# stevengiacalone/triceratops

Hardware: AMD Instinct MI355X
Metric: light-curve-point x sample evals/sec (higher is better)
Workload: dtype f64

## Files before the change

### include/trx_debug.h

```cpp
#ifndef TRX_DEBUG_H
#define TRX_DEBUG_H

#include "trx.h"

#ifdef __cplusplus
extern "C" {
#endif

int trx_set_rows_per_wave(int rows);
int trx_set_cell_packing_below(int n_time);
int trx_debug_batch_plan(long rows, int rows_per_wave, int taper, long* positions, int* rows_min);

int trx_set_supersample_tiers(int on);
int trx_set_stencil(int on);
int trx_set_skip_excluded(int on);
int trx_set_debug_node_counts(int on);
int trx_set_kepler_stepping(int on);

int trx_set_bounded_evaluation(int mode);
int trx_set_debug_bounded_lnl(int on);
int trx_set_debug_poison(int on);
int trx_set_debug_bug(int on);
int trx_set_probe_rows(int rows);
int trx_set_star_chain(int on);
int trx_set_row_order(int on);
int trx_debug_row_order(long* n_rows, long* segment_capacity, int* counts, int* lists, double* row_blocks);
int trx_set_whole_trips(int on);
int trx_set_one_sweep(int mode);
int trx_debug_whole_trips(long* whole, long* walked, int reset);
int trx_debug_chain_counts(long* chains, long* calls_in_chains, long* posterior_calls_in_chains, int reset);

int trx_debug_select_from_halfchi2(const double* halfchi2, const double* lnprior, const double* cols,
                                   const double* cols_pad, long n, long N, long n_total, int ncol, int twin, int K,
                                   int moments, double lnsigma, double* out_record, double* out_post_x,
                                   double* out_table, void* stream);

int trx_debug_capture_buffers(long* live, long* idle);

#ifdef __cplusplus
}
#endif
#endif
```

### triceratops_amd/_lib.py

```python
import ctypes
import os
import threading

import numpy as np
import torch

_HERE = os.path.dirname(os.path.abspath(__file__))
LIB_PATH = os.environ.get("TRX_LIB") or os.path.join(_HERE, "libtrx.so")
TESTING_LIB_PATH = os.environ.get("TRX_TESTING_LIB") or os.path.join(_HERE, "libtrx_testing.so")

MODEL_TP, MODEL_EB, MODEL_EB_TWIN, MODEL_RAW = 0, 1, 2, 3
FLAG_COMPANION_IS_HOST, FLAG_SCALAR_K, FLAG_FP32_MODEL, FLAG_EVALUATE_EXCLUDED = 1, 2, 4, 8
FLAG_ALL_SUBEXPOSURES, FLAG_NO_STENCIL, FLAG_COUNT_EVALUATIONS, FLAG_FULL_EVALUATION = 16, 32, 64, 128
FLAG_WEIGHT_MOMENTS = 256
N_PARAM = {MODEL_TP: 10, MODEL_EB: 11, MODEL_EB_TWIN: 11, MODEL_RAW: 9}
ERR_NTOTAL = 4

ABI_SYMBOLS = (
    "trx_lnl_batch", "trx_lnl_batch_weighted", "trx_flux_grid", "trx_chi2_grid", "trx_chi2_grid_weighted",
    "trx_chi2_grid_offset", "trx_chi2_grid_baseline", "trx_workspace_bytes",
    "trx_log_mean_exp", "trx_lnz_scenario", "trx_lnz_from_halfchi2", "trx_lnz_moments_from_halfchi2",
    "trx_posterior_from_halfchi2", "trx_grid_quantiles",
    "trx_lnl_batch_host", "trx_flux_grid_host",
    "trx_log_mean_exp_host", "trx_skipped_rows", "trx_pruned_rows",
    "trx_draw_scenario", "trx_draw_args_size", "trx_scenario_evidence", "trx_scenario_enqueue", "trx_star_enqueue",
    "trx_scenario_args_size", "trx_release_scratch", "trx_version", "trx_last_error", "trx_device_count",
)
WARP_SYMBOLS = ("trxw_hist_from_halfchi2",)
NOISE_SYMBOLS = ("trxn_chi2_grid_ou",)
MIX_SYMBOLS = ("trxm_chi2_grid_ou_mix",)
SHIFT_SYMBOLS = ("trxt_softmin_rows",)
ROBUST_SYMBOLS = ("trxr_chi2_grid_robust",)
GLS_SYMBOLS = ("trxg_chi2_grid_ou_baseline",)
SS_SYMBOLS = ("trxs_chi2_grid_ss2",)
DEBUG_SYMBOLS = (
    "trx_set_rows_per_wave", "trx_set_cell_packing_below", "trx_debug_batch_plan", "trx_set_supersample_tiers",
    "trx_set_stencil", "trx_set_skip_excluded", "trx_set_debug_node_counts", "trx_set_kepler_stepping",
    "trx_set_bounded_evaluation", "trx_set_debug_bounded_lnl", "trx_set_debug_poison", "trx_set_debug_bug",
    "trx_set_probe_rows", "trx_set_star_chain", "trx_debug_capture_buffers", "trx_debug_chain_counts",
    "trx_set_row_order", "trx_debug_row_order", "trx_set_whole_trips", "trx_debug_whole_trips", "trx_set_one_sweep",
    "trx_debug_select_from_halfchi2",
)


class TrxError(RuntimeError):
    pass


EXTRA_FLAGS = 0
CELL_PACKING_BELOW = 320
STATS = {"rows": 0, "cells": 0, "launches": 0, "native_calls": 0}
_stats_lock = threading.Lock()


def count_launch(rows, n_time):
    with _stats_lock:
        STATS["rows"] += rows
        STATS["cells"] += rows * n_time
        STATS["launches"] += 1
TRACE = None
TRACE_SAMPLE_ROWS = 128


def reset_stats():
    for k in STATS:
        STATS[k] = 0


def set_precision(mode):
    global EXTRA_FLAGS
    if mode not in ("fp64", "fp32"):
        raise ValueError("precision must be 'fp64' or 'fp32'")
    EXTRA_FLAGS = (EXTRA_FLAGS & ~FLAG_FP32_MODEL) | (FLAG_FP32_MODEL if mode == "fp32" else 0)

# ... 87 lines not shown
                                        _vp]
    L.trxt_softmin_rows.restype = c_int
    L.trxt_softmin_rows.argtypes = [_vp, c_long, c_long, c_int, _vp, c_int, _vp, _vp]
    L.trxr_chi2_grid_robust.restype = c_int
    L.trxr_chi2_grid_robust.argtypes = [_vp, _vp, _vp, c_int, c_long, _vp, c_double, c_int, _vp, c_double, c_double, c_double,
                                        _vp]
    L.trxg_chi2_grid_ou_baseline.restype = c_int
    L.trxg_chi2_grid_ou_baseline.argtypes = [_vp, _vp, c_int, c_long, _vp, c_double, c_int, _vp, _vp, _vp, _vp, _vp, c_int,
                                             _vp, _vp, _vp]
    L.trxs_chi2_grid_ss2.restype = c_int
    L.trxs_chi2_grid_ss2.argtypes = [_vp, _vp, c_int, c_long, _vp, c_double, c_int, _vp, _vp, _vp, _vp, _vp]
    L.trx_grid_quantiles.restype = c_int
    L.trx_grid_quantiles.argtypes = [_vp, c_long, c_int, _vp, _vp, c_long, _vp, c_int, _vp, _vp]
    L.trx_lnl_batch_host.restype = c_int
    L.trx_lnl_batch_host.argtypes = [c_int, c_int, _vp, _vp, c_int, c_double, _vp, c_long,
                                     c_double, c_int, _vp]
    L.trx_flux_grid_host.restype = c_int
    L.trx_flux_grid_host.argtypes = [c_int, c_int, _vp, c_int, _vp, c_long, c_double, c_int, _vp, _vp]
    L.trx_log_mean_exp_host.restype = c_int
    L.trx_log_mean_exp_host.argtypes = [_vp, c_long, c_long, _vp]
    L.trx_skipped_rows.restype = c_int
    L.trx_skipped_rows.argtypes = [ctypes.POINTER(ctypes.c_ulonglong), c_int]
    L.trx_pruned_rows.restype = c_int
    L.trx_pruned_rows.argtypes = [ctypes.POINTER(ctypes.c_ulonglong), c_int]
    L.trx_version.restype = ctypes.c_char_p
    L.trx_last_error.restype = ctypes.c_char_p
    L.trx_device_count.restype = c_int
    L.trx_testing = bool(testing)
    if testing:
        for name in ("trx_set_rows_per_wave", "trx_set_kepler_stepping", "trx_set_skip_excluded",
                     "trx_set_bounded_evaluation", "trx_set_debug_bounded_lnl", "trx_set_debug_poison",
                     "trx_set_debug_bug", "trx_set_star_chain", "trx_set_probe_rows", "trx_set_stencil",
                     "trx_set_supersample_tiers", "trx_set_debug_node_counts", "trx_set_cell_packing_below",
                     "trx_set_row_order", "trx_set_whole_trips", "trx_set_one_sweep"):
            fn = getattr(L, name)
            fn.restype = c_int
            fn.argtypes = [c_int]
        L.trx_debug_capture_buffers.restype = c_int
        L.trx_debug_capture_buffers.argtypes = [ctypes.POINTER(c_long), ctypes.POINTER(c_long)]
        L.trx_debug_row_order.restype = c_int
        L.trx_debug_row_order.argtypes = [ctypes.POINTER(c_long), ctypes.POINTER(c_long), _vp, _vp, _vp]
        L.trx_debug_whole_trips.restype = c_int
        L.trx_debug_whole_trips.argtypes = [ctypes.POINTER(c_long), ctypes.POINTER(c_long), c_int]
        L.trx_debug_select_from_halfchi2.restype = c_int
        L.trx_debug_select_from_halfchi2.argtypes = [_vp, _vp, _vp, _vp, c_long, c_long, c_long, c_int, c_int, c_int, c_int,
                                                     c_double, _vp, _vp, _vp, _vp]
    return L


def check(rc):
    if rc:
        msg = lib().trx_last_error().decode()
        if rc == ERR_NTOTAL:
            raise ValueError(msg)
        raise TrxError("libtrx error %d: %s" % (rc, msg))


def version():
    return lib().trx_version().decode()


_gpu_seen = False


def require_gpu():
    global _gpu_seen
    if _gpu_seen:
        return
    if not torch.cuda.is_available() or lib().trx_device_count() < 1:
        raise TrxError("triceratops_amd needs an AMD GPU (gfx950); none is visible and there is no "
# ... 475 lines not shown
```

### triceratops_amd/csrc/trx_cells.hpp

```cpp
#pragma once
#include <hip/hip_runtime.h>
#include <math.h>

#include <cstddef>
#include <cstdint>

#include "../../include/trx.h"
#include "trx_device.hpp"
#include "trx_internal.hpp"

namespace {

using namespace trx;

constexpr int MODE_LNL = 0;
constexpr int MODE_GRID = 1;

struct RowsArgs {
    int model, flags;
    const double* time;
    const double* flux;
    int n_time;
    double sigma;
    const double* params;
// ... 14 lines not shown
    int tl_off;
    int wave_off, wave_doubles;
    int probe_rows;
    int wave_floor;
    int wave_floor3;
    double* rowc;
    int* scan_list;
    unsigned long long* scan_count;
    const long* n_dev;
    const int* src_idx;
    long src_stride;
    int twin_cols;
    int dense;
    int forced_B;
    int prune;
    int pstride;
    int pstride3;
    double prune_c0;
    const double* prune_lp;
    int part;
    int split;
    int* surv_list;
    unsigned long long* surv_count;
    int* probe_list;
    unsigned long long* probe_count;
    TierHead tiers;
    const double* tier_xw;
    double s2, rs2, dS, rS;
    const double* inv_var;
    double sec_limit;
    int accumulate;
    int whole_trips;
    int one_sweep;
    int* order;
};

#ifndef TRX_CHAIN_MAX_BRANCHES
#define TRX_CHAIN_MAX_BRANCHES 24
#endif
struct BranchArgs {
    int model, flags, twin_cols, need_sec;
    const double* flux;
    double sigma, s2, rs2, prune_c0;
    const double* params;
    double* out;
    const long* n_dev;
    const int* src_idx;
    const double* prune_lp;
    double* scratch;
    unsigned long long* scan_count;
};
constexpr int kChainMaxBranches = TRX_CHAIN_MAX_BRANCHES;
struct BranchTab {
    BranchArgs b[kChainMaxBranches];
};
static_assert(sizeof(RowsArgs) + sizeof(BranchTab) + 16 <= 4096, "kernel argument buffer");

__device__ __forceinline__ double uniform(double v)
{
    const unsigned long long b = __double_as_longlong(v);
    const unsigned lo = __builtin_amdgcn_readfirstlane((unsigned)b);
    const unsigned hi = __builtin_amdgcn_readfirstlane((unsigned)(b >> 32));
    return __longlong_as_double(((unsigned long long)hi << 32) | lo);
}

__device__ __forceinline__ long uniform_long(long v)
// ... 20 lines not shown
    return __builtin_amdgcn_mbcnt_hi((unsigned)(m >> 32), __builtin_amdgcn_mbcnt_lo((unsigned)m, 0u));
}

#ifdef TRX_PHASE_TIMERS
__device__ unsigned long long g_phase_cycles[8];
#define TRX_TICK(var) const unsigned long long var = __builtin_readcyclecounter()
#define TRX_TOCK(slot, from) tm[slot] += __builtin_readcyclecounter() - (from)
#else
#define TRX_TICK(var)
#define TRX_TOCK(slot, from)
#endif

#ifdef TRX_TAIL_TIMERS
constexpr int kTailWaves = 1 << 17;
__device__ unsigned long long g_tail[4] = {~0ull, 0ull, 0ull, 0ull};
__device__ unsigned long long g_tail_finish[kTailWaves];
#endif

constexpr int kStatShards = 256, kStatPad = 16;
__device__ unsigned long long g_row_stats[2][kStatShards][kStatPad];
__device__ __forceinline__ void add_row_stat(int which, unsigned count)
{
    if (count) atomicAdd(&g_row_stats[which][(blockIdx.x + 41u * blockIdx.y) & (kStatShards - 1)][0], (unsigned long long)count);
}

#ifdef TRX_TESTING
__device__ unsigned long long g_trip_stats[2][kStatShards][kStatPad];
__device__ __forceinline__ void add_trip_stat(int which, unsigned count)
{
    if (count) atomicAdd(&g_trip_stats[which][(blockIdx.x + 41u * blockIdx.y) & (kStatShards - 1)][0], (unsigned long long)count);
}
__device__ __forceinline__ bool whole_trips_on(const RowsArgs& a) { return a.whole_trips != 0; }
__device__ __forceinline__ bool one_sweep_on(const RowsArgs& a, bool lnl) { return a.one_sweep >= (lnl ? 1 : 2); }
#define TRX_TRIP_STAT(var) ++var
#else
__device__ __forceinline__ bool whole_trips_on(const RowsArgs&) { return true; }
__device__ __forceinline__ bool one_sweep_on(const RowsArgs&, bool lnl) { return lnl; }
#define TRX_TRIP_STAT(var)
#endif

__device__ __forceinline__ double k_rule(double k, bool scalar_rule)
{
    if (scalar_rule) { if (fabs(k - 1.0) < 1e-6) k *= 0.999; }
    else             { if ((k - 1.0) < 1e-6) k *= 0.999; }
    return k;
}

#ifndef TRX_BATCH_WAVES
#define TRX_BATCH_WAVES 4
#endif

constexpr int kBatchWaves = TRX_BATCH_WAVES;
__host__ __device__ constexpr int cells_waves(bool long_rows) { return long_rows ? 1 : kBatchWaves; }
#ifndef TRX_TIER_LDS
#define TRX_TIER_LDS(PRUNE, LONG) true
#endif
#ifndef TRX_ATAN_TAB
#define TRX_ATAN_TAB(PRUNE, LONG) (((PRUNE) && !(LONG)) ? 2 : 1)
#endif
#ifndef TRX_LONG_ROWS_IN_LDS
#define TRX_LONG_ROWS_IN_LDS 0
#endif
#ifndef TRX_CARRY_CELLS
#define TRX_CARRY_CELLS 1
#endif
#ifndef TRX_CELLS_WAVES_PER_EU
#define TRX_CELLS_WAVES_PER_EU 4
#endif
#ifndef TRX_LAZY_TIERS
#define TRX_LAZY_TIERS 1
// ... 494 lines not shown
            double m = secnan[lane] ? NAN : secmin[lane];
            m = (m + ysec) / (1.0 + ysec);
            const double secdepth = 1.0 - (m + fdil) / (1.0 + fdil);
            a.rowc[row * kRowDoubles + (kRowDoubles - 1)] =
                (WT ? !(secdepth >= a.sec_limit) : (secdepth < 1.5 * a.sigma)) ? 0.0 : 1.0;
            if (a.out_sec) a.out_sec[row] = secdepth;
        }
        __syncthreads();
    }
}

template <int E, bool WT = false>
__global__ __launch_bounds__(64) void sec_scan_kernel(RowsArgs a)
{
    sec_scan_body<E, WT>(a);
}

struct BranchMap {
    unsigned char id[TRX_CHAIN_MAX_BRANCHES];
};
__global__ __launch_bounds__(64) void sec_scan_kernel_star(RowsArgs common, BranchTab bt, BranchMap map)
{
    const RowsArgs a = star_args(common, bt, 0, (int)map.id[blockIdx.y]);
    if (!a.need_sec) return;
    sec_scan_body<8>(a);
}
static_assert(offsetof(RowC, excl) == (kRowDoubles - 1) * sizeof(double), "excl is the last field of RowC");

struct CellState {
    double sE[64], cE[64];
    double t[64];
    double facc[64];
    unsigned meta[64];
    unsigned short rel[64];
};
struct StencilState {
    double fc[64 + ((kStM + 7) & ~7)];
    double stw[(2 * kStM + 1 + 7) & ~7];
};
constexpr int kCentreNode = 1023;

__device__ __forceinline__ double fp32_model_slack(double lb, int n_probed, double rs2)
{
    return 1e-5 * sqrt(2.0 * (double)n_probed * rs2 * fmax(lb, 0.0));
}

template <int BITS>
__device__ __forceinline__ int lane_prefix(int cnt, int& total)
{
    int off = 0;
    total = 0;
#pragma unroll
    for (int b = 0; b < BITS; ++b) {
        const unsigned long long m = __ballot((cnt >> b) & 1);
        off += lanes_below(m) << b;
        total += __popcll(m) << b;
    }
    return off;
}

__device__ __forceinline__ long row_order_at(const int* __restrict__ order, long v, long n, int lane)
{
    const int cnt = order[lane * kOrderStride];
    int incl = cnt;
#pragma unroll
    for (int o = 1; o < 64; o <<= 1) {
        const int up = __shfl_up(incl, o, 64);
        if (lane >= o) incl += up;
    }
    const long first = (long)(incl - cnt);
    const unsigned long long below = __ballot(cnt >= 0 && first <= v);
    const int seg = __popcll(below) - 1;
// ... 400 lines not shown
                    const double dMc = reduce_2pi(phase);
                    const double slack = 1e-15 * fabs(phase);
                    const RowC& cw = rows[rr];
                    inw = in_window(cw.wlo - slack, cw.whi + slack, dMc) && !mask_bit(skipmask, rr);
                    if (MODE == MODE_GRID && (!inw || a.debug_nodes))
                        a.out[(size_t)base * n_time + cell] = a.debug_nodes ? 0.0 : hmout[rr];
                    if (LONG && MODE == MODE_LNL && !inw && phase_no == 0) {
                        const double d = fl[j] - 1.0;
                        lacc = fma(d * d, WT ? wl[j] : rs2, lacc);
                    }
                    if (PRUNE) {
                        if (!LONG && inw && phase_no == 0) {
                            const double d = fl[j] - 1.0;
                            __hip_atomic_fetch_add(&hrem[rr], (d * d) * rs2, __ATOMIC_RELAXED, __HIP_MEMORY_SCOPE_WORKGROUP);
                        }
                        if (nphase == 2) {
                            const bool probe = (j % pstride) == (pstride >> 1);
                            inw = inw && (probe == (phase_no == 0));
                        }
                    }
                }
                const unsigned long long mw = __ballot(inw);
                if (inw) winlist[nw + lanes_below(mw)] = (unsigned short)(cell - win0);
                nw += __popcll(mw);
            }
            wave_sync();
            TRX_TOCK(1, t_p1);
            constexpr bool kOneSweep = TRX_ONE_SWEEP && (LONG || TRX_ONE_SWEEP_BATCH) && !PRUNE;
            const bool one = kOneSweep && one_sweep_on(a, MODE == MODE_LNL);
            int nheavy = 0;
            for (int sweep = 0; sweep < (one ? 1 : 2); ++sweep) {
            const int count = sweep ? nheavy : nw;
            const bool halo = ST && sweep == 0 && st_radius > 0.0;
            int carry_j = 0;
            unsigned long long carry_ok = 0;
            int ncarry = 0;
            for (int w0 = 0, step = 64; w0 < count || (kCarry && ncarry > 0); w0 += step) {
                TRX_TICK(t_plan);
                TRX_CENSUS_ADD(sweep ? kCenChunk1 : kCenChunk0, 1);
                bool owned = true;
                const bool carried = kCarry && lane < ncarry;
                if (kCarry) step = 64 - ncarry;
                const int csrc = (lane + 64 - ncarry) & 63;
                const unsigned cmeta = carried ? cs.meta[csrc] : 0u;
                bool valid = carried ? (cmeta & 0x20000u) != 0 : (w0 + lane - ncarry) < count;
                int rel = (int)*(carried ? &cs.rel[csrc] : &winlist[valid ? (w0 + lane - ncarry) : (count - 1)]);
                bool last_chunk = false;
                if (ST && halo) {
                    last_chunk = w0 + 64 >= count;
                    step = last_chunk ? 64 : 64 - kStM;
                    owned = lane < step;
                    if (w0 > 0 && lane < kStM) ss.fc[lane] = ss.fc[kStM + (64 - 2 * kStM) + lane];
                    wave_sync();
                }
                const int cell = win0 + rel;
                int rr = 0, j = cell;
                if (!LONG) {
                    rr = (int)(((float)cell + 0.5f) * inv_nt);
                    rr = rr < nb ? rr : nb - 1;
                    j = cell - rr * n_time;
                }
                const double t = tl[j];
                double fobs = 0.0;
                if (LONG && MODE == MODE_LNL) fobs = fl[j];
                double wobs = rs2;
                if (LONG && WT) wobs = wl[j];
                CellPlan pl;
                if (carried) {
                    pl.n = (int)(cmeta >> 18); pl.tier = (int)((cmeta >> 8) & 0xffu) - 1;
                    pl.sE = cs.sE[csrc]; pl.cE = cs.cE[csrc];
                    pl.anchored = (cmeta & 0x10000u) != 0;
                } else if (valid) {
                    const RowC& c = (LONG && !TRX_LONG_ROWS_IN_LDS) ? cu : rows[rr];
#ifndef TRX_PLAN_FULL_SOLVE
                    if (LONG && sweep == 1) pl = plan_all_subexposures<PRUNE>(c, t, a.S);
                    else
#endif
                    pl = plan_cell<false, PRUNE, TRX_TIER_LDS(PRUNE, LONG), kLazyTiers>(c, t, a.exptime, a.S, a.tiers, a.use_tiers != 0,
                                                                                        (ST && sweep == 0) ? st_radius : 0.0, thead);
                    if (STEP && !pl.anchored && pl.n > 0) {
                        kepler_full(c.nmot * (t - c.t0) + c.Mtr, c.e, pl.sE, pl.cE);
                        pl.anchored = true;
                    }
                }
                bool planned = valid;
                if (sweep == 0 && a.use_tiers) {
                    const bool heavy = valid && !pl.lazy && pl.tier < 0 && pl.n > 0;
                    if (one) {
                        planned = valid && !heavy;
                    } else {
                        const unsigned long long mh = __ballot(heavy && owned);
                        if (heavy && owned) winlist[nheavy + lanes_below(mh)] = (unsigned short)rel;
                        if (heavy) { pl.n = 0; valid = false; planned = false; }
                        nheavy += __popcll(mh);
                    }
                }
                int tier = pl.tier;
                int nodes = (valid && owned) ? pl.n : 0;
                bool st = false, centre = false;
                if (ST && sweep == 0) {
                    const int jleft = __shfl(carry_j, 64 - 2 * kStM + lane, 64), jhere = __shfl(j, lane - kStM, 64);
                    const int jm = (lane < kStM) ? jleft : jhere;
                    const int jp = __shfl(j, lane + kStM, 64);
                    const unsigned long long mok = __ballot(planned);
                    const unsigned long long left = (carry_ok >> (64 - 2 * kStM)) & ((1ull << kStM) - 1ull);
                    const bool inner = (lane >= kStM || (halo && w0 > 0)) && lane + kStM < 64;
                    constexpr unsigned long long kAll = (1ull << (2 * kStM + 1)) - 1ull;
                    const unsigned long long field = (lane >= kStM) ? (mok >> (lane - kStM)) : (((mok << kStM) | left) >> lane);
                    st = inner && owned && planned && pl.n > 0 && pl.st_ok && jm == j - kStM && jp == j + kStM &&
                         (field & kAll) == kAll;
                    const unsigned long long mst = __ballot(st);
                    unsigned long long dil = mst;
#pragma unroll
                    for (int i = 1; i <= kStM; ++i) dil |= (mst << i) | (mst >> i);
                    centre = planned && ((dil >> lane) & 1ull);
                    const unsigned long long mnext = __ballot(planned && pl.n > 0 && pl.st_ok) >> (64 - kStM);
                    const int kk = lane - (64 - 2 * kStM);
                    if (halo && !last_chunk && planned && !centre && kk >= 0 && kk < kStM && (mnext & ((2ull << kk) - 1ull)) != 0) {
                        if (pl.n > 0) centre = true;
                        else ss.fc[kStM + lane] = 1.0;
                    }
                    if (st) nodes = 0;
                    carry_j = j;
                    carry_ok = mok;
                    if (kLazyTiers) {
                        const bool need = pl.lazy && nodes > 0;
                        if (__any(need)) {
                            if (need) {
                                const RowC& c = (LONG && !TRX_LONG_ROWS_IN_LDS) ? cu : rows[rr];
                                plan_tiers(c, a.exptime, pl, thead);
                                tier = pl.tier;
                                nodes = pl.n;
                            }
                        }
                    }
                }
                const bool direct = kLazyTiers && ST && sweep == 0 && !__any(nodes > 0);
                if (direct) {
                    if (centre) {
                        const RowC& c = (LONG && !TRX_LONG_ROWS_IN_LDS) ? cu : rows[rr];
                        const double ce = pl.cE - c.e;
                        const double X = fma(c.ax, ce, c.bx * pl.sE);
                        const double Y = fma(c.ay, ce, c.by * pl.sE);
                        const double yc = Y * c.cosi;
                        const double z2 = fma(X, X, yc * yc);
                        const double opp = 1.0 + c.k;
                        double f = 1.0;
                        if (Y >= 0.0 && z2 < opp * opp) {
                            const Limb L{c.cle, c.cld, c.ced};
                            f = disc_flux<FP32, TRX_ATAN_TAB(PRUNE, LONG)>(sqrt_fast(z2), c.k, L, atab);
                        } else if (z2 != z2) {
                            f = z2;
                        }
                        ss.fc[kStM + lane] = f;
                    }
                    wave_sync();
                }
                if (kCarry) wave_sync();
                if (!direct) {
                    cs.sE[lane] = pl.sE; cs.cE[lane] = pl.cE;
                    cs.t[lane] = t;
                    cs.facc[lane] = 0.0;
                    cs.meta[lane] = (unsigned)rr | ((unsigned)(tier + 1) << 8) | (pl.anchored ? 0x10000u : 0u) |
                                    (valid ? 0x20000u : 0u) | ((unsigned)pl.n << 18);
                    if (kCarry) cs.rel[lane] = (unsigned short)rel;
                }
                TRX_TOCK(2, t_plan);
                TRX_TICK(t_a);
                int ldone = 64;
                const int ncells = __popcll(__ballot(nodes > 0 || (ST && centre)));
                const bool by_cells = one && a.S < kCellsPairs;
                int per = ncells > 0 ? kCellsPairs / ncells - (ST ? 1 : 0) : kCellsPairs;
                per = per > 1000 ? 1000 : (per < 1 ? 1 : per);
                if (by_cells) per = kCellsPairs;
                int lane0 = ncells > 0 ? 0 : 64;
                for (int s0 = 0; !direct && (by_cells ? lane0 < 64 : __any(s0 < nodes || (ST && s0 == 0 && centre)));
                     s0 += by_cells ? 0 : per) {
                    int cnt = nodes - s0;
                    cnt = cnt < 0 ? 0 : (cnt > per ? per : cnt);
                    TRX_CENSUS_ADD(kCenPass, 1);
                    int extra = (ST && s0 == 0 && centre) ? 1 : 0;
                    if (by_cells && lane < lane0) { cnt = 0; extra = 0; }
                    int total;
                    int off;
                    if (one) off = (a.S + 1 < 32) ? lane_prefix<5>(cnt + extra, total) : lane_prefix<10>(cnt + extra, total);
                    else off = (sweep == 0 && a.use_tiers) ? lane_prefix<4>(cnt + extra, total) : lane_prefix<10>(cnt + extra, total);
                    if (by_cells) {
// ... 25 lines not shown
                            const int d = (int)pdesc[p];
                            const int h = d & 63;
                            const bool at_centre = ST && (d >> 6) == kCentreNode;
                            const int s = at_centre ? 0 : s0 + (d >> 6);
                            const unsigned meta = cs.meta[h];
                            const RowC& c = (LONG && !TRX_LONG_ROWS_IN_LDS) ? cu : rows[meta & 0xffu];
                            const int ht = (int)((meta >> 8) & 0xffu) - 1;
                            double sE = cs.sE[h], cE = cs.cE[h];
                            if (!at_centre) {
                                const double frac = (ht < 0) ? fma((double)(s + 1) - 0.5, a.rS, -0.5)
                                                             : tier_xw[2 * (ht * kTierMaxNodes + s)];
                                const double dM = c.nmot * (a.exptime * frac);
                                bool have = false;
                                if (STEP && (meta & 0x10000u)) have = kepler_step<PRUNE>(dM, c.e, sE, cE);
                                if (!have) {
                                    TRX_CENSUS_ADD(kCenKeplerFullPair, 1);
                                    kepler_full(c.nmot * ((cs.t[h] + a.exptime * frac) - c.t0) + c.Mtr, c.e, sE, cE);
                                }
                            }
                            const double ce = cE - c.e;
                            const double X = fma(c.ax, ce, c.bx * sE);
                            const double Y = fma(c.ay, ce, c.by * sE);
                            const double yc = Y * c.cosi;
                            const double z2 = fma(X, X, yc * yc);
                            const double opp = 1.0 + c.k;
                            double f = 1.0;
                            if (Y >= 0.0 && z2 < opp * opp) {
                                const Limb L{c.cle, c.cld, c.ced};
                                f = disc_flux<FP32, TRX_ATAN_TAB(PRUNE, LONG)>(sqrt_fast(z2), c.k, L, atab);
                            } else if (z2 != z2) {
                                f = z2;
                            }
                            if (at_centre) {
                                ss.fc[kStM + h] = f;
                            } else {
                                const double term = (ht < 0) ? f : tier_xw[2 * (ht * kTierMaxNodes + s) + 1] * (1.0 - f);
                                if (ht < 0 || term != 0.0)
                                    __hip_atomic_fetch_add(&cs.facc[h], term, __ATOMIC_RELAXED, __HIP_MEMORY_SCOPE_WORKGROUP);
                            }
                        }
                    }
                    wave_sync();
                }
                TRX_TOCK(3, t_a);
                TRX_TICK(t_rest);
                if (MODE == MODE_GRID && a.debug_nodes) {
                    const int spent = nodes + ((ST && centre) ? 1 : 0);
                    if (spent > 0 && lane < ldone) atomicAdd(&a.out[(size_t)base * n_time + cell], (double)spent);
                } else if (valid && owned && lane < ldone) {
                    const RowC& c = (LONG && !TRX_LONG_ROWS_IN_LDS) ? cu : rows[rr];
                    double fsum = cs.facc[lane];
                    if (ST && st) {
                        fsum = 0.0;
#pragma unroll
                        for (int i = -kStM; i <= kStM; ++i) fsum = fma(ss.stw[i + kStM], 1.0 - ss.fc[kStM + lane + i], fsum);
                    }
                    const double deficit = (pl.n == 0) ? 0.0 : ((ST && st) ? fsum : ((tier < 0) ? 1.0 - fsum / a.dS : fsum));
                    const RowC& cd = rows[rr];
                    const double m = fma(-deficit, cd.rdil, 1.0);
                    if (MODE == MODE_GRID) {
                        a.out[(size_t)base * n_time + cell] = m;
                    } else {
                        if (LONG) {
                            const double d = fobs - m;
                            lacc = fma(d * d, wobs, lacc);
                            nonflat = nonflat || (m != 1.0);
                        } else {
                            const double f = fl[j];
                            const double contrib = ((1.0 - m) * ((f - m) + (f - 1.0))) * (WT ? wl[j] : rs2);
                            if (contrib != 0.0)
                                __hip_atomic_fetch_add(&hacc[rr], contrib, __ATOMIC_RELAXED, __HIP_MEMORY_SCOPE_WORKGROUP);
                            if (PRUNE && nphase == 2 && phase_no == 0) {
                                const double d1 = f - 1.0;
                                __hip_atomic_fetch_add(&hrem[rr], -(d1 * d1) * rs2, __ATOMIC_RELAXED, __HIP_MEMORY_SCOPE_WORKGROUP);
                            }
                        }
                    }
                }
                if (kCarry) ncarry = 64 - ldone;
                TRX_TOCK(5, t_rest);
            }
            }
            wave_sync();
            if (PRUNE && nphase == 2 && phase_no == 0) {
                const double* hdr_b = a.rowc + n * kRowDoubles;
                const double hmin_run = __hip_atomic_load(&hdr_b[kHdrHmin], __ATOMIC_RELAXED, __HIP_MEMORY_SCOPE_AGENT);
                const double xmax_run = __hip_atomic_load(&hdr_b[kHdrXmax], __ATOMIC_RELAXED, __HIP_MEMORY_SCOPE_AGENT);
                if (LONG) {
                    double lb = 0.5 * wave_sum(lacc);
                    lb -= fma(1e-9, fabs(lb), 1e-9);
                    if (FP32) lb -= fp32_model_slack(lb, n_time / pstride + 1, rs2);
                    const double lp0 = hlp[0];
                    long_dead = hmout[0] == 1.0 && lb > hmin_run && (a.prune_c0 - lb + lp0) < xmax_run - 90.0;
                    if (long_dead) {
                        if (lane == 0) a.out[base] = lb;
                        ++n_pruned;
                        break;
                    }
                } else {
                    bool dead = false;
                    if (lane < nb && !mask_bit(skipmask, lane)) {
                        double lb = 0.5 * (flat_sum + hacc[lane] - hrem[lane]);
                        lb -= fma(1e-9, fabs(lb) + flat_sum, 1e-9);
                        if (FP32) lb -= fp32_model_slack(lb, n_time / pstride + 1, rs2);
                        dead = hmout[lane] == 1.0 && lb > hmin_run && (a.prune_c0 - lb + lp_row) < xmax_run - 90.0;
#ifdef TRX_PRUNE_NEVER_DEAD
                        dead = false;
#endif
                        if (dead) hrem[lane] = lb;
                    }
// ... 258 lines not shown
```

### triceratops_amd/csrc/trx_kernels.hip

```cpp
#include <hip/hip_runtime.h>
#include <math.h>
#include <stdio.h>
#include <stdlib.h>
#include <string.h>

#include <atomic>
#include <cstddef>
#include <cstdint>
#include <map>
#include <mutex>
#include <type_traits>
#include <utility>
#include <vector>

#include "../../include/trx.h"
#include "../../include/trx_noise.h"
#include "../../include/trx_mix.h"
#include "../../include/trx_shift.h"
#include "../../include/trx_robust.h"
#include "../../include/trx_gls.h"
#include "../../include/trx_ss.h"
#include "trx_device.hpp"
#include "trx_internal.hpp"
#include "trx_knobs.hpp"
// ... 223 lines not shown
    else      hipLaunchKernelGGL((cells_kernel<MODE, true, false, LONG, ST, PRUNE, WT>), g, block, lds, st, a);
}

template <int MODE>
void launch_pruned(const RowsArgs& a, hipStream_t st, bool long_rows, bool fp32, unsigned grid, size_t lds)
{
    if constexpr (MODE == MODE_LNL) {
        if (long_rows) launch_cells_kernel<MODE_LNL, true, false, true, false>(true, fp32, grid, lds, st, a);
        else           launch_cells_kernel<MODE_LNL, false, false, true, false>(true, fp32, grid, lds, st, a);
    }
}

bool short_rows(int n_time) { return n_time > 0 && n_time < knob_cells_below(); }

struct CellsPlan {
    bool long_rows, prune, split, fp32, step;
    size_t lds;
    unsigned grid_main;
    unsigned grid_pilot;
    unsigned grid_rowc;
    unsigned grid_scan;
    unsigned grid_screen;
    bool passes;
    int probe_B;
    size_t probe_lds;
    int probe_wave_doubles;
};

#ifndef TRX_PROBE_FP32
#define TRX_PROBE_FP32 1
#endif
constexpr bool kProbeFp32 = TRX_PROBE_FP32 != 0;

template <int MODE>
int plan_cells(RowsArgs& a, bool long_rows, CellsPlan& P)
{
    a.forced_B = knob_rows_per_wave();
    a.B = long_rows ? 1 : batch_rows(a.n_dev ? -1 : a.n, a.n_time, a.forced_B);
    a.s2 = a.sigma * a.sigma;
    a.rs2 = 1.0 / a.s2;
    a.dS = (double)a.S;
    a.rS = 1.0 / a.dS;
    a.nbatch = 8 * batch_plan(a.n, a.B).P;
    a.debug_bug = knob_debug_bug();
    a.whole_trips = knob_whole_trips();
    a.one_sweep = knob_one_sweep();
    a.mark_unwritten = (MODE == MODE_LNL && !a.inv_var) ? 1 : 0;
    bool tiers_ok = false;
    if (tier_device(a.S, a.tiers, &a.tier_xw, &tiers_ok)) return fail(TRX_ERR_HIP, "tier table upload failed%s", "", 0);
    a.use_tiers = tiers_ok && knob_tiers() && !(a.flags & TRX_FLAG_ALL_SUBEXPOSURES);
    const int prune_mode = (a.flags & TRX_FLAG_FULL_EVALUATION) ? 0 : (a.prune == 2 ? 2 : knob_bounded());
    const bool prune = MODE == MODE_LNL && a.prune && knob_kepler_stepping() &&
                       (prune_mode == 2 || (prune_mode == 1 && long_rows)) &&
                       (long_rows || (long)a.B * a.n_time <= (long)kCellsWindowBatch) &&
                       a.n_time >= kProbeMinPoints;
    a.prune = prune ? 1 : 0;
    static const int probe_cells = (int)env_long("TRX_PROBE_CELLS", kProbeCells);
    a.pstride = prune ? (a.n_time / probe_cells > 1 ? a.n_time / probe_cells : 2) : 1;
    static const int third_stride = (int)env_long("TRX_THIRD_STRIDE", kThirdStride);
    a.pstride3 = (prune && third_stride > 1 && a.n_time >= 4 * third_stride) ? third_stride : 0;
    a.use_stencil = (!prune && long_rows && a.use_tiers && a.exptime > 0.0 && a.S >= 8 && a.n_time >= 64 &&
                     knob_stencil() && !(a.flags & TRX_FLAG_NO_STENCIL)) ? 1 : 0;
    a.skip_excl = knob_skip_excluded() && !(a.flags & TRX_FLAG_EVALUATE_EXCLUDED);
    a.need_sec = (a.model == TRX_MODEL_EB && MODE == MODE_LNL) ||
                 ((a.model == TRX_MODEL_EB || a.model == TRX_MODEL_EB_TWIN) && a.out_sec != nullptr);
    if (a.inv_var && !(a.sec_limit < INFINITY)) a.need_sec = 0;
    static_assert((kCellsPairs + kCellsWindowLong) % 4 == 0 && (kCellsPairs + kCellsWindowBatch) % 4 == 0 &&
                  sizeof(CellState) % 8 == 0 && sizeof(StencilState) % 8 == 0, "8-byte alignment of the LDS arrays");
    const size_t tables = (size_t)(2 * kTiers * kTierMaxNodes + kAtanRanges * kAtanCols + kTierHeadDoubles) * sizeof(double);
    auto wave_bytes = [&](bool long_variant) -> size_t {
        return (size_t)a.B * (kRowDoubles + 4) * sizeof(double)
             + (kCellsPairs + cells_window(long_variant)) * sizeof(unsigned short) + sizeof(CellState)
             + (long_variant ? sizeof(StencilState) : 0);
    };
    a.tl_off = (int)(tables / sizeof(double));
    size_t shared = tables + (long_rows ? 0 : (size_t)(a.inv_var ? 3 : 2) * a.n_time * sizeof(double));
    size_t lds = shared + cells_waves(long_rows) * wave_bytes(long_rows);
    if (lds > 64 * 1024) {
        long_rows = true;
        a.B = 1;
        a.nbatch = a.n;
        shared = tables;
        lds = shared + wave_bytes(true);
    }
    a.wave_off = (int)(shared / sizeof(double));
    a.wave_doubles = (int)(wave_bytes(long_rows) / sizeof(double));
#ifdef TRX_NO_SPLIT
    const bool split = false;
#else
    const bool split = prune && !long_rows;
#endif
    a.split = split ? 1 : 0;
    P.probe_B = a.B;
    P.probe_lds = lds;
    P.probe_wave_doubles = a.wave_doubles;
    a.probe_rows = 0;
    a.wave_floor = a.wave_floor3 = 3200;
    if (split && knob_probe_rows() != 1) {
        const int forced = knob_probe_rows();
        const int per_row = a.n_time / a.pstride + 1;
        const size_t fixed = (kCellsPairs + cells_window(false)) * sizeof(unsigned short) + sizeof(CellState);
        const size_t room = (32 * 1024 - shared) / cells_waves(false);
        int B2 = room > fixed ? (int)((room - fixed) / ((kRowDoubles + 4) * sizeof(double))) : a.B;
        if (forced > 1) B2 = forced;
        if (B2 > kCellsMaxRows) B2 = kCellsMaxRows;
        if (B2 * per_row > cells_window(false)) B2 = cells_window(false) / per_row;
        if ((long)B2 * a.n_time > 65535) B2 = 65535 / a.n_time;
// ... 1046 lines not shown
}

int trx_set_supersample_tiers(int on)
{
    g_knob_tiers = on ? 1 : 0;
    return TRX_OK;
}

int trx_set_debug_node_counts(int on)
{
    g_knob_debug_nodes = on ? 1 : 0;
    return TRX_OK;
}

int trx_set_row_order(int on)
{
    g_knob_row_order = on ? 1 : 0;
    return TRX_OK;
}

int trx_set_whole_trips(int on)
{
    g_knob_whole_trips = on ? 1 : 0;
    return TRX_OK;
}

int trx_set_one_sweep(int mode)
{
    if (mode < 0 || mode > 2) return fail(TRX_ERR_ARG, "trx_set_one_sweep: mode must be 0, 1 or 2%s (got %ld)", "", (long)mode);
    g_knob_one_sweep = mode;
    return TRX_OK;
}

int trx_debug_whole_trips(long* whole, long* walked, int reset)
{
    static unsigned long long host[2][kStatShards][kStatPad];
    static std::mutex mu;
    std::lock_guard<std::mutex> lock(mu);
    TRX_HIP(hipDeviceSynchronize());
    TRX_HIP(hipMemcpyFromSymbol(host, HIP_SYMBOL(g_trip_stats), sizeof(host), 0));
    long sum[2] = {0, 0};
    for (int w = 0; w < 2; ++w)
        for (int i = 0; i < kStatShards; ++i) sum[w] += (long)host[w][i][0];
    if (whole) *whole = sum[0];
    if (walked) *walked = sum[1];
    if (reset) {
        memset(host, 0, sizeof(host));
        TRX_HIP(hipMemcpyToSymbol(HIP_SYMBOL(g_trip_stats), host, sizeof(host), 0));
    }
    return TRX_OK;
}

int trx_debug_row_order(long* n_rows, long* segment_capacity, int* counts, int* lists, double* row_blocks)
{
    if (!t_last_order || !t_last_rowc) return fail(TRX_ERR_ARG, "trx_debug_row_order: no ordered launch yet%s", "", 0);
    const long n = t_last_order_rows, cap = order_cap(n);
    if (n_rows) *n_rows = n;
    if (segment_capacity) *segment_capacity = cap;
    if (!counts && !lists && !row_blocks) return TRX_OK;
    TRX_HIP(hipDeviceSynchronize());
    if (counts) {
        std::vector<int> raw((size_t)kOrderSegs * kOrderStride);
        TRX_HIP(hipMemcpy(raw.data(), t_last_order, raw.size() * sizeof(int), hipMemcpyDeviceToHost));
        for (int sgm = 0; sgm < kOrderSegs; ++sgm) counts[sgm] = raw[(size_t)sgm * kOrderStride];
    }
    if (lists)
// ... 86 lines not shown
```

### triceratops_amd/csrc/trx_knobs.hpp

```cpp
#pragma once
#include <stdlib.h>

#ifdef TRX_TESTING
#include <atomic>
#endif

namespace trx {

#ifdef TRX_TESTING
inline int knob_env_int(const char* name, int dflt)
{
    const char* e = name ? getenv(name) : nullptr;
    return (e && *e) ? atoi(e) : dflt;
}
inline long env_long(const char* name, long dflt)
{
    const char* e = getenv(name);
    return (e && *e) ? atol(e) : dflt;
}
inline double env_double(const char* name, double dflt)
{
    const char* e = getenv(name);
    return (e && *e) ? atof(e) : dflt;
}
#define TRX_KNOB(name, dflt, env)                                              \
    inline std::atomic<int> g_knob_##name{knob_env_int(env, dflt)};           \
    inline int knob_##name() { return g_knob_##name.load(std::memory_order_relaxed); }
#else
constexpr long env_long(const char*, long dflt) { return dflt; }
constexpr double env_double(const char*, double dflt) { return dflt; }
#define TRX_KNOB(name, dflt, env) \
    constexpr int knob_##name() { return dflt; }
#endif

TRX_KNOB(rows_per_wave, 0, nullptr)
TRX_KNOB(probe_rows, 0, "TRX_PROBE_ROWS")
TRX_KNOB(kepler_stepping, 1, nullptr)
TRX_KNOB(tiers, 1, nullptr)
TRX_KNOB(bounded, 2, "TRX_BOUNDED")
TRX_KNOB(bounded_lnl, 0, nullptr)
TRX_KNOB(skip_excluded, 1, nullptr)
TRX_KNOB(stencil, 1, nullptr)
TRX_KNOB(debug_nodes, 0, nullptr)
TRX_KNOB(cells_below, 320, nullptr)
TRX_KNOB(debug_bug, 0, nullptr)
TRX_KNOB(poison, 0, nullptr)
TRX_KNOB(star_chain, 1, "TRX_STAR_CHAIN")
TRX_KNOB(row_order, 1, nullptr)
TRX_KNOB(whole_trips, 1, nullptr)
TRX_KNOB(one_sweep, 1, nullptr)

#undef TRX_KNOB

}
```

Baseline: 51.39 billion.

## Advance stencil sweep by full 64-lane chunks, deferring boundary cells to next chunk

In the single-sweep stencil path, chunks used to advance by 64 minus the stencil radius, so the halo lanes were re-planned in every chunk. Chunks now advance by a full 64 lanes. Cells near the chunk boundary whose stencil needs the next chunk's centre values are held as pending, with their observed flux and weight parked in LDS, and are finished by the next chunk. This removes the re-evaluation of overlapping halo cells in the LNL path by default, at the cost of extra ballots, LDS bookkeeping and more complex boundary logic.

```diff
diff --git a/include/trx_debug.h b/include/trx_debug.h
--- a/include/trx_debug.h
+++ b/include/trx_debug.h
@@ -27,6 +27,8 @@
 int trx_debug_row_order(long* n_rows, long* segment_capacity, int* counts, int* lists, double* row_blocks);
 int trx_set_whole_trips(int on);
 int trx_set_one_sweep(int mode);
+int trx_set_full_chunks(int mode);
+long trx_debug_cells_lds_one_row(void);
 int trx_debug_whole_trips(long* whole, long* walked, int reset);
 int trx_debug_chain_counts(long* chains, long* calls_in_chains, long* posterior_calls_in_chains, int reset);
 
diff --git a/profiles/full_chunks/evals_per_cell.py b/profiles/full_chunks/evals_per_cell.py
--- /dev/null
+++ b/profiles/full_chunks/evals_per_cell.py
@@ -0,0 +1,25 @@
+import os
+import sys
+
+import numpy as np
+
+sys.path.insert(0, os.path.join(os.path.dirname(os.path.abspath(__file__)), "..", ".."))
+from triceratops_amd import _lib, synth
+
+_lib.use_testing_library(True)
+L = _lib.lib()
+rng = np.random.default_rng(synth.SEED)
+t_d = _lib.dev(synth.time_grid(2000))
+rows = [_lib.dev(synth.family_rows(rng, fam, 512)) for fam in synth.FAMILIES]
+assert L.trx_set_one_sweep(2) == 0
+for mode in (0, 2):
+    assert L.trx_set_full_chunks(mode) == 0
+    total = cells = 0.0
+    for (name, model, is_host, has_comp), r in zip(synth.FAMILIES, rows):
+        flags = (_lib.FLAG_COMPANION_IS_HOST if is_host else 0) | _lib.FLAG_COUNT_EVALUATIONS
+        c, _ = _lib.flux_grid(model, flags, t_d, r, synth.EXPTIME, synth.NSAMPLES, False)
+        total += float(c.sum())
+        cells += float(c.numel())
+    print("trx_set_full_chunks(%d): %.6f model evaluations per cell (%d families x 512 rows x 2000 points)"
+          % (mode, total / cells, len(rows)))
+assert L.trx_set_one_sweep(1) == 0 and L.trx_set_full_chunks(1) == 0
diff --git a/triceratops_amd/_lib.py b/triceratops_amd/_lib.py
--- a/triceratops_amd/_lib.py
+++ b/triceratops_amd/_lib.py
@@ -39,7 +39,7 @@
     "trx_set_bounded_evaluation", "trx_set_debug_bounded_lnl", "trx_set_debug_poison", "trx_set_debug_bug",
     "trx_set_probe_rows", "trx_set_star_chain", "trx_debug_capture_buffers", "trx_debug_chain_counts",
     "trx_set_row_order", "trx_debug_row_order", "trx_set_whole_trips", "trx_debug_whole_trips", "trx_set_one_sweep",
-    "trx_debug_select_from_halfchi2",
+    "trx_set_full_chunks", "trx_debug_cells_lds_one_row", "trx_debug_select_from_halfchi2",
 )
 
 
@@ -193,10 +193,12 @@
                      "trx_set_bounded_evaluation", "trx_set_debug_bounded_lnl", "trx_set_debug_poison",
                      "trx_set_debug_bug", "trx_set_star_chain", "trx_set_probe_rows", "trx_set_stencil",
                      "trx_set_supersample_tiers", "trx_set_debug_node_counts", "trx_set_cell_packing_below",
-                     "trx_set_row_order", "trx_set_whole_trips", "trx_set_one_sweep"):
+                     "trx_set_row_order", "trx_set_whole_trips", "trx_set_one_sweep", "trx_set_full_chunks"):
             fn = getattr(L, name)
             fn.restype = c_int
             fn.argtypes = [c_int]
+        L.trx_debug_cells_lds_one_row.restype = c_long
+        L.trx_debug_cells_lds_one_row.argtypes = []
         L.trx_debug_capture_buffers.restype = c_int
         L.trx_debug_capture_buffers.argtypes = [ctypes.POINTER(c_long), ctypes.POINTER(c_long)]
         L.trx_debug_row_order.restype = c_int
diff --git a/triceratops_amd/csrc/trx_cells.hpp b/triceratops_amd/csrc/trx_cells.hpp
--- a/triceratops_amd/csrc/trx_cells.hpp
+++ b/triceratops_amd/csrc/trx_cells.hpp
@@ -70,6 +70,7 @@
     int accumulate;
     int whole_trips;
     int one_sweep;
+    int full_chunks;
     int* order;
 };
 
@@ -156,10 +157,12 @@
 }
 __device__ __forceinline__ bool whole_trips_on(const RowsArgs& a) { return a.whole_trips != 0; }
 __device__ __forceinline__ bool one_sweep_on(const RowsArgs& a, bool lnl) { return a.one_sweep >= (lnl ? 1 : 2); }
+__device__ __forceinline__ bool full_chunks_on(const RowsArgs& a, bool lnl) { return a.full_chunks >= (lnl ? 1 : 2); }
 #define TRX_TRIP_STAT(var) ++var
 #else
 __device__ __forceinline__ bool whole_trips_on(const RowsArgs&) { return true; }
 __device__ __forceinline__ bool one_sweep_on(const RowsArgs&, bool lnl) { return lnl; }
+__device__ __forceinline__ bool full_chunks_on(const RowsArgs&, bool lnl) { return lnl; }
 #define TRX_TRIP_STAT(var)
 #endif
 
@@ -720,12 +723,16 @@
     double t[64];
     double facc[64];
     unsigned meta[64];
-    unsigned short rel[64];
+    union {
+        unsigned short rel[64];
+        double held[2 * kStM];
+    };
 };
 struct StencilState {
-    double fc[64 + ((kStM + 7) & ~7)];
-    double stw[(2 * kStM + 1 + 7) & ~7];
+    double fc[64 + 2 * kStM];
+    double stw[2 * kStM + 1];
 };
+constexpr int kFcB = 2 * kStM;
 constexpr int kCentreNode = 1023;
 
 __device__ __forceinline__ double fp32_model_slack(double lb, int n_probed, double rs2)
@@ -1192,8 +1199,11 @@
             for (int sweep = 0; sweep < (one ? 1 : 2); ++sweep) {
             const int count = sweep ? nheavy : nw;
             const bool halo = ST && sweep == 0 && st_radius > 0.0;
+            const bool full = halo && one && full_chunks_on(a, MODE == MODE_LNL);
+            const bool lend = halo && !full;
             int carry_j = 0;
             unsigned long long carry_ok = 0;
+            unsigned pendm = 0;
             int ncarry = 0;
             for (int w0 = 0, step = 64; w0 < count || (kCarry && ncarry > 0); w0 += step) {
                 TRX_TICK(t_plan);
@@ -1206,11 +1216,17 @@
                 bool valid = carried ? (cmeta & 0x20000u) != 0 : (w0 + lane - ncarry) < count;
                 int rel = (int)*(carried ? &cs.rel[csrc] : &winlist[valid ? (w0 + lane - ncarry) : (count - 1)]);
                 bool last_chunk = false;
-                if (ST && halo) {
+                const unsigned pend_prev = pendm;
+                if (ST && full) {
+                    const int ln = lanes_below(~0ull);
+                    if (w0 > 0 && ln < 2 * kStM) ss.fc[ln] = ss.fc[64 + ln];
+                    wave_sync();
+                }
+                if (ST && lend) {
                     last_chunk = w0 + 64 >= count;
                     step = last_chunk ? 64 : 64 - kStM;
                     owned = lane < step;
-                    if (w0 > 0 && lane < kStM) ss.fc[lane] = ss.fc[kStM + (64 - 2 * kStM) + lane];
+                    if (w0 > 0 && lane < kStM) ss.fc[kFcB - kStM + lane] = ss.fc[kFcB + (64 - 2 * kStM) + lane];
                     wave_sync();
                 }
                 const int cell = win0 + rel;
@@ -1259,30 +1275,58 @@
                 int nodes = (valid && owned) ? pl.n : 0;
                 bool st = false, centre = false;
                 if (ST && sweep == 0) {
-                    const int jleft = __shfl(carry_j, 64 - 2 * kStM + lane, 64), jhere = __shfl(j, lane - kStM, 64);
+                    const int lsrc = full ? 64 - kStM : 64 - 2 * kStM;
+                    const int jleft = __shfl(carry_j, lsrc + lane, 64), jhere = __shfl(j, lane - kStM, 64);
                     const int jm = (lane < kStM) ? jleft : jhere;
-                    const int jp = __shfl(j, lane + kStM, 64);
+                    int jp = __shfl(j, lane + kStM, 64);
                     const unsigned long long mok = __ballot(planned);
-                    const unsigned long long left = (carry_ok >> (64 - 2 * kStM)) & ((1ull << kStM) - 1ull);
-                    const bool inner = (lane >= kStM || (halo && w0 > 0)) && lane + kStM < 64;
-                    constexpr unsigned long long kAll = (1ull << (2 * kStM + 1)) - 1ull;
+                    const unsigned long long left = (carry_ok >> lsrc) & ((1ull << kStM) - 1ull);
+                    int nnext = 0;
+                    const int j_last = __builtin_amdgcn_readlane(j, 63);
+                    if (full && w0 + 64 < count) {
+                        const int more = count - (w0 + 64) < kStM ? count - (w0 + 64) : kStM;
+                        if (win0 + (int)winlist[w0 + 63 + more] == j_last + more) nnext = more;
+                    }
+                    constexpr unsigned kAll = (1u << (2 * kStM + 1)) - 1u;
+                    unsigned want = kAll;
+                    bool inner = (lane >= kStM || (halo && w0 > 0)) && lane + kStM < 64;
+                    if (nnext > 0) {
+                        const int over = lanes_below(~0ull) - (63 - kStM);
+                        if (over > 0 && over <= nnext) {
+                            jp = j_last + over;
+                            want = kAll >> over;
+                            inner = true;
+                        }
+                    }
                     const unsigned long long field = (lane >= kStM) ? (mok >> (lane - kStM)) : (((mok << kStM) | left) >> lane);
                     st = inner && owned && planned && pl.n > 0 && pl.st_ok && jm == j - kStM && jp == j + kStM &&
-                         (field & kAll) == kAll;
+                         ((unsigned)field & kAll) == want;
                     const unsigned long long mst = __ballot(st);
                     unsigned long long dil = mst;
 #pragma unroll
                     for (int i = 1; i <= kStM; ++i) dil |= (mst << i) | (mst >> i);
                     centre = planned && ((dil >> lane) & 1ull);
+                    pendm = (unsigned)(mst >> (64 - kStM));
+                    bool has_value = centre;
+                    if (full) {
+                        const bool owes = pend_prev != 0 && lanes_below(~0ull) < 32 - __clz((int)pend_prev);
+                        if (__any(owes && !centre)) {
+                            if (owes) {
+                                if (pl.n > 0) centre = true;
+                                else if (!centre) ss.fc[kFcB + lane] = 1.0;
+                                has_value = true;
+                            }
+                        }
+                    }
                     const unsigned long long mnext = __ballot(planned && pl.n > 0 && pl.st_ok) >> (64 - kStM);
                     const int kk = lane - (64 - 2 * kStM);
-                    if (halo && !last_chunk && planned && !centre && kk >= 0 && kk < kStM && (mnext & ((2ull << kk) - 1ull)) != 0) {
+                    if (lend && !last_chunk && planned && !centre && kk >= 0 && kk < kStM && (mnext & ((2ull << kk) - 1ull)) != 0) {
                         if (pl.n > 0) centre = true;
-                        else ss.fc[kStM + lane] = 1.0;
+                        else ss.fc[kFcB + lane] = 1.0;
                     }
                     if (st) nodes = 0;
                     carry_j = j;
-                    carry_ok = mok;
+                    carry_ok = full ? __ballot(has_value) : mok;
                     if (kLazyTiers) {
                         const bool need = pl.lazy && nodes > 0;
                         if (__any(need)) {
@@ -1312,7 +1356,7 @@
                         } else if (z2 != z2) {
                             f = z2;
                         }
-                        ss.fc[kStM + lane] = f;
+                        ss.fc[kFcB + lane] = f;
                     }
                     wave_sync();
                 }
@@ -1404,7 +1448,7 @@
                                 f = z2;
                             }
                             if (at_centre) {
-                                ss.fc[kStM + h] = f;
+                                ss.fc[kFcB + h] = f;
                             } else {
                                 const double term = (ht < 0) ? f : tier_xw[2 * (ht * kTierMaxNodes + s) + 1] * (1.0 - f);
                                 if (ht < 0 || term != 0.0)
@@ -1416,26 +1460,37 @@
                 }
                 TRX_TOCK(3, t_a);
                 TRX_TICK(t_rest);
+                const int lq = lanes_below(~0ull) - (64 - kStM);
+                const bool mine_pending = ST && st && pendm != 0 && lq >= 0;
+                bool adopt = mine_pending;
+                unsigned left_over = 0u;
+                if (ST && pend_prev != pendm) {
+                    const bool prev_here = lq >= 0 && ((pend_prev >> lq) & 1u) != 0;
+                    adopt = prev_here && (mine_pending || !valid);
+                    left_over = (unsigned)(__ballot(prev_here && !adopt) >> (64 - kStM));
+                }
                 if (MODE == MODE_GRID && a.debug_nodes) {
                     const int spent = nodes + ((ST && centre) ? 1 : 0);
                     if (spent > 0 && lane < ldone) atomicAdd(&a.out[(size_t)base * n_time + cell], (double)spent);
-                } else if (valid && owned && lane < ldone) {
+                } else if ((valid && owned && lane < ldone && !mine_pending) || adopt) {
                     const RowC& c = (LONG && !TRX_LONG_ROWS_IN_LDS) ? cu : rows[rr];
                     double fsum = cs.facc[lane];
-                    if (ST && st) {
+                    if (ST && (st || adopt)) {
+                        const double* fcl = &ss.fc[kFcB + (adopt ? lq - kStM : lane)];
                         fsum = 0.0;
 #pragma unroll
-                        for (int i = -kStM; i <= kStM; ++i) fsum = fma(ss.stw[i + kStM], 1.0 - ss.fc[kStM + lane + i], fsum);
-                    }
-                    const double deficit = (pl.n == 0) ? 0.0 : ((ST && st) ? fsum : ((tier < 0) ? 1.0 - fsum / a.dS : fsum));
+                        for (int i = -kStM; i <= kStM; ++i) fsum = fma(ss.stw[i + kStM], 1.0 - fcl[i], fsum);
+                    }
+                    const double deficit = (ST && adopt) ? fsum
+                                         : ((pl.n == 0) ? 0.0 : ((ST && st) ? fsum : ((tier < 0) ? 1.0 - fsum / a.dS : fsum)));
                     const RowC& cd = rows[rr];
                     const double m = fma(-deficit, cd.rdil, 1.0);
                     if (MODE == MODE_GRID) {
-                        a.out[(size_t)base * n_time + cell] = m;
+                        a.out[(size_t)base * n_time + ((ST && adopt) ? win0 + (int)winlist[w0] - kStM + lq : cell)] = m;
                     } else {
                         if (LONG) {
-                            const double d = fobs - m;
-                            lacc = fma(d * d, wobs, lacc);
+                            const double d = ((ST && adopt) ? cs.held[lq] : fobs) - m;
+                            lacc = fma(d * d, (ST && WT && adopt) ? cs.held[kStM + lq] : wobs, lacc);
                             nonflat = nonflat || (m != 1.0);
                         } else {
                             const double f = fl[j];
@@ -1448,6 +1503,27 @@
                             }
                         }
                     }
+                }
+                if (ST && left_over != 0 && !(MODE == MODE_GRID && a.debug_nodes)) {
+                    const int q = lanes_below(~0ull);
+                    if (q < kStM && ((left_over >> q) & 1u)) {
+                        const int jq = win0 + (int)winlist[w0] - kStM + q;
+                        double fsum = 0.0;
+#pragma unroll
+                        for (int i = -kStM; i <= kStM; ++i) fsum = fma(ss.stw[i + kStM], 1.0 - ss.fc[kFcB - kStM + q + i], fsum);
+                        const double m = fma(-fsum, rows[0].rdil, 1.0);
+                        if (MODE == MODE_GRID) {
+                            a.out[(size_t)base * n_time + jq] = m;
+                        } else {
+                            const double d = cs.held[q] - m;
+                            lacc = fma(d * d, WT ? cs.held[kStM + q] : rs2, lacc);
+                            nonflat = nonflat || (m != 1.0);
+                        }
+                    }
+                }
+                if (ST && MODE == MODE_LNL && mine_pending) {
+                    cs.held[lq] = fobs;
+                    if (WT) cs.held[kStM + lq] = wobs;
                 }
                 if (kCarry) ncarry = 64 - ldone;
                 TRX_TOCK(5, t_rest);
diff --git a/triceratops_amd/csrc/trx_kernels.hip b/triceratops_amd/csrc/trx_kernels.hip
--- a/triceratops_amd/csrc/trx_kernels.hip
+++ b/triceratops_amd/csrc/trx_kernels.hip
@@ -279,6 +279,18 @@
 #endif
 constexpr bool kProbeFp32 = TRX_PROBE_FP32 != 0;
 
+constexpr size_t cells_tables_bytes()
+{
+    return (size_t)(2 * kTiers * kTierMaxNodes + kAtanRanges * kAtanCols + kTierHeadDoubles) * sizeof(double);
+}
+constexpr size_t cells_wave_bytes(int B, bool long_variant)
+{
+    return (size_t)B * (kRowDoubles + 4) * sizeof(double)
+         + (kCellsPairs + cells_window(long_variant)) * sizeof(unsigned short) + sizeof(CellState)
+         + (long_variant ? sizeof(StencilState) : 0);
+}
+static_assert(cells_tables_bytes() + cells_wave_bytes(1, true) <= 160 * 1024 / 16, "LDS of the one-row workgroup");
+
 template <int MODE>
 int plan_cells(RowsArgs& a, bool long_rows, CellsPlan& P)
 {
@@ -292,6 +304,7 @@
     a.debug_bug = knob_debug_bug();
     a.whole_trips = knob_whole_trips();
     a.one_sweep = knob_one_sweep();
+    a.full_chunks = knob_full_chunks();
     a.mark_unwritten = (MODE == MODE_LNL && !a.inv_var) ? 1 : 0;
     bool tiers_ok = false;
     if (tier_device(a.S, a.tiers, &a.tier_xw, &tiers_ok)) return fail(TRX_ERR_HIP, "tier table upload failed%s", "", 0);
@@ -314,12 +327,8 @@
     if (a.inv_var && !(a.sec_limit < INFINITY)) a.need_sec = 0;
     static_assert((kCellsPairs + kCellsWindowLong) % 4 == 0 && (kCellsPairs + kCellsWindowBatch) % 4 == 0 &&
                   sizeof(CellState) % 8 == 0 && sizeof(StencilState) % 8 == 0, "8-byte alignment of the LDS arrays");
-    const size_t tables = (size_t)(2 * kTiers * kTierMaxNodes + kAtanRanges * kAtanCols + kTierHeadDoubles) * sizeof(double);
-    auto wave_bytes = [&](bool long_variant) -> size_t {
-        return (size_t)a.B * (kRowDoubles + 4) * sizeof(double)
-             + (kCellsPairs + cells_window(long_variant)) * sizeof(unsigned short) + sizeof(CellState)
-             + (long_variant ? sizeof(StencilState) : 0);
-    };
+    const size_t tables = cells_tables_bytes();
+    auto wave_bytes = [&](bool long_variant) -> size_t { return cells_wave_bytes(a.B, long_variant); };
     a.tl_off = (int)(tables / sizeof(double));
     size_t shared = tables + (long_rows ? 0 : (size_t)(a.inv_var ? 3 : 2) * a.n_time * sizeof(double));
     size_t lds = shared + cells_waves(long_rows) * wave_bytes(long_rows);
@@ -1432,6 +1441,18 @@
     return TRX_OK;
 }
 
+int trx_set_full_chunks(int mode)
+{
+    if (mode < 0 || mode > 2) return fail(TRX_ERR_ARG, "trx_set_full_chunks: mode must be 0, 1 or 2%s (got %ld)", "", (long)mode);
+    g_knob_full_chunks = mode;
+    return TRX_OK;
+}
+
+long trx_debug_cells_lds_one_row(void)
+{
+    return (long)(cells_tables_bytes() + cells_wave_bytes(1, true));
+}
+
 int trx_debug_whole_trips(long* whole, long* walked, int reset)
 {
     static unsigned long long host[2][kStatShards][kStatPad];
diff --git a/triceratops_amd/csrc/trx_knobs.hpp b/triceratops_amd/csrc/trx_knobs.hpp
--- a/triceratops_amd/csrc/trx_knobs.hpp
+++ b/triceratops_amd/csrc/trx_knobs.hpp
@@ -49,6 +49,7 @@
 TRX_KNOB(row_order, 1, nullptr)
 TRX_KNOB(whole_trips, 1, nullptr)
 TRX_KNOB(one_sweep, 1, nullptr)
+TRX_KNOB(full_chunks, 1, nullptr)
 
 #undef TRX_KNOB
 
```

New measurement: 52.85 billion, median of 6. 2.8% higher.
